# MCG-NJU/LinK

Hardware: AMD Instinct MI355X
Metric: voxels/s through one LinK (3x7)^3 block, 100k active voxels C=64 (higher is better)
Workload: dtype f32

## Files before the change

link_amd/csrc/dense_batch_impl.h:

```cpp
#include <stdlib.h>

#include <type_traits>
#include <vector>

#include "dense_batch_common.h"
#include "dense_gather.h"
#include "dense_io.h"

namespace DC_IO_NS {
using namespace link;

#include "dense_k1_impl.h"
#include "dense_k2_cfg.h"
#include "dense_gather_quad_impl.h"

static_assert(DC_ST_AUX == 16, "the S rows must leave the L2 (sc1) for the in-launch hand-off K1 -> K2");

struct dc_bt_frame_t {
  const void *feats; const int4 *coords; int4 *slots; uint32_t *cnt; int32_t *cell_n; int32_t *vcell; float *S; int32_t *hdr;
  void *out; int64_t n;
};
struct dc_bt_frames_t { dc_bt_frame_t f[DC_BT_MAX]; };
struct dc_bt_par_t {
  const float *w_pre, *pre_ln_w, *pre_ln_b, *w_pos, *ln_w, *ln_b;
// ... 48 lines not shown
    const link_dc_grid_t g = a->g;
    const int n = (int)a->fr.f[f].n;
    const int4 *__restrict__ coords = a->fr.f[f].coords;
    int32_t *__restrict__ vcell = a->fr.f[f].vcell;
    int32_t *__restrict__ hdr = a->fr.f[f].hdr;
    const __amdgpu_buffer_rsrc_t r_slots = dc_rsrc(a->fr.f[f].slots, (uint32_t)((int64_t)g.vp * g.k * 16));
    const __amdgpu_buffer_rsrc_t r_cnt = dc_rsrc(a->fr.f[f].cnt, (uint32_t)(g.vp * 4));
    if (j == 0 && threadIdx.x == 0) hdr[LINK_HDR_NVALID] = n;
    _Pragma("unroll 1") for (int k = 0; k < 4; k++) {
      const int v = (4 * j + k) * 64 + (int)threadIdx.x;
      if (v >= n) break;
      const int4 rc = coords[v];
      const unsigned ux = (unsigned)(floordiv(rc.x, g.s) - g.lo[0]), uy = (unsigned)(floordiv(rc.y, g.s) - g.lo[1]);
      const unsigned uz = (unsigned)(floordiv(rc.z, g.s) - g.lo[2]), ub = (unsigned)(rc.w - g.lo[3]);
      const bool inside = ux < (unsigned)g.dim[0] && uy < (unsigned)g.dim[1] && uz < (unsigned)g.dim[2] && ub < (unsigned)g.dim[3];
      if (!inside) atomicOr(&hdr[LINK_HDR_STATUS_ACC], 1);
      const int pcell = inside ? dc_cell(g, (int)ux, (int)uy, (int)uz, (int)ub) : 0;
      const int rank = __builtin_amdgcn_raw_ptr_buffer_atomic_add_i32(1, r_cnt, pcell ? (uint32_t)pcell * 4u : DC_OOB, 0, 0);
      const bool full = pcell != 0 && rank >= g.k;
      if (full) atomicOr(&hdr[LINK_HDR_STATUS_ACC], 2);
      const bool keep = pcell != 0 && !full;
      st16i_c<true>(r_slots, keep ? dc_slot(g, pcell, rank) * 16u : DC_OOB, make_int4(rc.x, rc.y, rc.z, v));
      vcell[v] = keep ? pcell : 0;
    }
    asm volatile("s_waitcnt vmcnt(0)" ::: "memory");
    if (threadIdx.x == 0) __hip_atomic_fetch_add(&a->sync[bt_ins(f)], 1, __ATOMIC_RELAXED, __HIP_MEMORY_SCOPE_AGENT);
  }
#endif
}

template <int OP, int NB>
__global__ void __launch_bounds__(64 * DC_K1_NW, DC_K1_WAVES) k_dc_batch_k1(dc_bt_frames_t fr, dc_bt_par_t p, link_dc_grid_t g, int nframes,
                                                                           int cpw, int nranges, int wpf, int32_t *__restrict__ sync) {
  constexpr int C = 64;
  extern __shared__ __attribute__((aligned(16))) char smem_raw[];
  const int tid = threadIdx.x, lane = tid & 63;
  bool w_big = false, th_big = false;
  dc_k1_stage<C, OP>(smem_raw, p.w_pre, p.pre_ln_w, p.pre_ln_b, p.w_pos, nullptr, p.cg, 1.0f, g, tid, w_big, th_big);
  w_big = DC_K1_SPLIT ? (__syncthreads_or(w_big) != 0) : (__syncthreads(), false);
  const bool th_slow = DC_THETA_BOUND ? __syncthreads_or(th_big) != 0 : false;
  const int Vi = g.dim[0] * g.dim[1] * g.dim[2] * g.dim[3];
  const int x = (int)(__builtin_amdgcn_s_getreg((4 - 1) << 11 | 0 << 6 | 20) & 7u);
  const int per = (nranges + 7) >> 3;
  const int lo = x * per;
  const int mine = (lo + per < nranges ? lo + per : nranges) - lo;
  if (mine <= 0) return;
  const int total = nframes * mine;
  int32_t *cur = &sync[bt_k1cur(x)];
  int t_next = 0;
  if (lane == 0) t_next = __hip_atomic_fetch_add(cur, 1, __ATOMIC_RELAXED, __HIP_MEMORY_SCOPE_AGENT);
  int pend_f = -1;
  int ins_known = -1;
  for (;;) {
    const int t = __builtin_amdgcn_readfirstlane(t_next);
    if (t >= total) break;
    const unsigned long long tp0 = DC_BT_PROF ? __builtin_amdgcn_s_memrealtime() : 0;
    const int f = t / mine, i = lo + (t - f * mine);
    if (lane == 0) t_next = __hip_atomic_fetch_add(cur, 1, __ATOMIC_RELAXED, __HIP_MEMORY_SCOPE_AGENT);
    const dc_bt_frame_t &F = fr.f[f];
    int ins_a = wpf, ins_b = wpf;
    if (lane == 0) {
      if (f > ins_known) ins_a = __hip_atomic_load(&sync[bt_ins(f)], __ATOMIC_RELAXED, __HIP_MEMORY_SCOPE_AGENT);
      if (f + 1 < nframes && f + 1 > ins_known) ins_b = __hip_atomic_load(&sync[bt_ins(f + 1)], __ATOMIC_RELAXED, __HIP_MEMORY_SCOPE_AGENT);
    }
    const int c_begin = i * cpw;
    const int c_end = (c_begin + cpw < Vi) ? c_begin + cpw : Vi;
    int pc_f, nv_f;
    int4 rf0, rf1, rf2, rf3;
    if (f <= ins_known) dc_k1_prefetch<true>(pc_f, nv_f, rf0, rf1, rf2, rf3, g, F.slots, F.cnt, c_begin, c_end, lane);
    asm volatile("s_waitcnt vmcnt(0)" ::: "memory");
    if (pend_f >= 0 && lane == 0) __hip_atomic_fetch_add(&sync[bt_k1(pend_f)], 1, __ATOMIC_RELAXED, __HIP_MEMORY_SCOPE_AGENT);
    pend_f = f;
    if (f > ins_known) {
      if (__builtin_amdgcn_readfirstlane(ins_a) < wpf && !bt_wait_ge(sync, bt_ins(f), wpf)) return;
      ins_known = f;
      dc_k1_prefetch<true>(pc_f, nv_f, rf0, rf1, rf2, rf3, g, F.slots, F.cnt, c_begin, c_end, lane);
    }
    if (f + 1 < nframes && f + 1 > ins_known && __builtin_amdgcn_readfirstlane(ins_b) >= wpf) ins_known = f + 1;
    if (i == 0 && lane == 0) {
      F.hdr[LINK_HDR_STATUS] = __hip_atomic_load(&F.hdr[LINK_HDR_STATUS_ACC], __ATOMIC_RELAXED, __HIP_MEMORY_SCOPE_AGENT);
      __hip_atomic_store(&F.hdr[LINK_HDR_STATUS_ACC], 0, __ATOMIC_RELAXED, __HIP_MEMORY_SCOPE_AGENT);
    }
    const unsigned long long tp1 = DC_BT_PROF ? __builtin_amdgcn_s_memrealtime() : 0;
    dc_k1_range<C, OP, NB, false, true, DC_BT_K1_WRITEBACK != 0>(smem_raw, F.feats, F.slots, F.cnt, F.cell_n, p.w_pre, 1.0f, p.eps, F.n, g, false, F.S, nullptr,
                                        nullptr, c_begin, c_end, pc_f, nv_f, rf0, rf1, rf2, rf3, w_big, th_slow, i, 0, 0);
    if (DC_BT_PROF && lane == 0) bt_row(p.dbg1, (unsigned long long)f * nranges + i, (unsigned long long)f, (unsigned long long)i, tp0, tp1, __builtin_amdgcn_s_memrealtime(), (unsigned long long)(blockIdx.x * 4 + (tid >> 6)));
  }
  asm volatile("s_waitcnt vmcnt(0)" ::: "memory");
#if DC_BT_RELEASE_FENCE
  __builtin_amdgcn_fence(__ATOMIC_RELEASE, "agent");
  asm volatile("s_waitcnt vmcnt(0)" ::: "memory");
#endif
  if (pend_f >= 0 && lane == 0) __hip_atomic_fetch_add(&sync[bt_k1(pend_f)], 1, __ATOMIC_RELAXED, __HIP_MEMORY_SCOPE_AGENT);
}

struct dc_bt_k2_args_t {
  dc_bt_frames_t fr;
  dc_bt_par_t p;
  link_dc_grid_t g;
  int nframes, txn, tyn, zsplit, nwg, k1_target;
  int32_t *sync;
};

template <int OP, int R>
__global__ void __launch_bounds__(256 + 64 * (DC_K2Q_CW + (DC_K2Q_PMAP ? 1 : 0)), 4) k_dc_batch_k2(dc_bt_k2_args_t args_by_value) {
  (void)args_by_value;
#if defined(__HIP_DEVICE_COMPILE__)
  static_assert(DC_K2Q_PMAP == 1, "the mapper wave draws the items");
  typedef const __attribute__((address_space(4))) dc_bt_k2_args_t *args_ptr_t;
  constexpr unsigned CTL_THREAD = 256 + 64 * DC_K2Q_CW;
  __shared__ int s_ctl[4];
  const int x = (int)(__builtin_amdgcn_s_getreg((4 - 1) << 11 | 0 << 6 | 20) & 7u);
  if (threadIdx.x == CTL_THREAD) {
    args_ptr_t a = (args_ptr_t)__builtin_amdgcn_kernarg_segment_ptr();
    int32_t *sy = a->sync;
    const int per = (a->nwg + 7) >> 3;
    if (DC_BT_PROF)
      bt_row(a->p.dbg2, (unsigned long long)a->nframes * (8 * per) + blockIdx.x, 9999, 0, __builtin_amdgcn_s_memrealtime(), 0, 0, blockIdx.x);
    const int t = __hip_atomic_fetch_add(&sy[bt_cursor(x)], 1, __ATOMIC_RELAXED, __HIP_MEMORY_SCOPE_AGENT);
    s_ctl[2] = __hip_atomic_fetch_add(&sy[bt_cursor(x)], 1, __ATOMIC_RELAXED, __HIP_MEMORY_SCOPE_AGENT);
    s_ctl[3] = x;
    int f = t < a->nframes * per ? t / per : -1;
    if (f >= 0 && !bt_wait_ge(sy, bt_k1(f), a->k1_target)) f = -1;
    s_ctl[0] = f; s_ctl[1] = f >= 0 ? (t - f * per) * 8 + x : 0;
  }
  __syncthreads();
  for (;;) {
    args_ptr_t a = (args_ptr_t)__builtin_amdgcn_kernarg_segment_ptr();
    asm volatile("" : "+s"(a));
    const int f = __builtin_amdgcn_readfirstlane(s_ctl[0]), bid = __builtin_amdgcn_readfirstlane(s_ctl[1]);
    if (f < 0) break;
    const unsigned long long tq0 = DC_BT_PROF ? __builtin_amdgcn_s_memrealtime() : 0;
    __syncthreads();
    {
      const link_dc_grid_t g = a->g;
      unsigned tidx = threadIdx.x;
      asm volatile("" : "+v"(tidx));
      dc_k2q_body<OP, R, false, true>(a->fr.f[f].S, a->fr.f[f].cell_n, a->fr.f[f].slots, a->p.w_pos, nullptr, a->p.ln_w, a->p.ln_b, a->p.cg,
                                      1.0f, a->p.eps, a->fr.f[f].n, g, a->txn, a->tyn, a->zsplit, a->nwg, a->fr.f[f].out, nullptr, bid, tidx);
    }
    if (threadIdx.x == CTL_THREAD) {
      const unsigned long long tq1 = DC_BT_PROF ? __builtin_amdgcn_s_memrealtime() : 0;
      int32_t *sy = a->sync;
      const int per = (a->nwg + 7) >> 3;
      const int t = s_ctl[2], xc = s_ctl[3];
      int fn = t < a->nframes * per ? t / per : -1;
      if (fn >= 0) {
        s_ctl[2] = __hip_atomic_fetch_add(&sy[bt_cursor(xc)], 1, __ATOMIC_RELAXED, __HIP_MEMORY_SCOPE_AGENT);
        if (!bt_wait_ge(sy, bt_k1(fn), a->k1_target)) fn = -1;
      }
      s_ctl[0] = fn; s_ctl[1] = fn >= 0 ? (t - fn * per) * 8 + xc : 0;
      if (DC_BT_PROF) bt_row(a->p.dbg2, (unsigned long long)f * (8 * per) + bid, (unsigned long long)f, (unsigned long long)bid, tq0, tq1, __builtin_amdgcn_s_memrealtime(), (unsigned long long)blockIdx.x);
    }
    __syncthreads();
  }
#endif
}


template <int OP, int R>
static int batch_launch(const dc_bt_host_t &c, const dc_bt_frames_t &fr, const dc_bt_par_t &p, const link_dc_grid_t &g, const link_elk_desc_t &d,
                        int nframes, int64_t nmax, bool strips) {
  using K1 = dc_k1_cfg<64, OP>;
  using KQ = dc_k2q_cfg<OP, R>;
  constexpr int LDS_GRAN = 1280, LDS_GRANS = 128, K1_STATIC = 256, K2_STATIC = 16;
  constexpr int k1_lds = 65 * LDS_GRAN - K1_STATIC;
  constexpr int k2_lds = KQ::LDS_BYTES;
// ... 51 lines not shown
```

link_amd/csrc/dense_fused_impl.h:

```cpp
#pragma once
#include <type_traits>

#include "dense_gather.h"
#include "dense_io.h"

namespace DC_IO_NS {
using namespace link;

#include "dense_k1_impl.h"

template <int C, int OP, int NB, bool PIPE, bool WB = true>
static int launch_k1p(const link_dc_buffers_t *b, const link_dc_grid_t &g, const link_elk_desc_t &d, int64_t n,
                     bool warm, hipStream_t st) {
  using K = dc_k1_cfg<C, OP>;
  const int64_t vi = (int64_t)g.dim[0] * g.dim[1] * g.dim[2] * g.dim[3];
  int64_t waves = (int64_t)(b->tune.k1_wgs > 0 ? b->tune.k1_wgs : 512) * 4;
  int cpw = (int)((vi + waves - 1) / waves);
  if (cpw < 1) cpw = 1;
  const int64_t wgs = (vi + (int64_t)cpw * K::NW - 1) / ((int64_t)cpw * K::NW);
  int k1_pad = b->tune.k1_lds_pad;
  k1_pad = k1_pad < 0 ? 0 : (k1_pad > 16384 ? 16384 : k1_pad);
  const int lds_k1 = K::LDS_BYTES + k1_pad <= 160 * 1024 ? K::LDS_BYTES + k1_pad : K::LDS_BYTES;
  if (lds_k1 > 64 * 1024)
    (void)hipFuncSetAttribute(reinterpret_cast<const void *>(&k_dc_premix_modsum<C, OP, NB, PIPE, WB>),
                              hipFuncAttributeMaxDynamicSharedMemorySize, lds_k1);
  hipLaunchKernelGGL((k_dc_premix_modsum<C, OP, NB, PIPE, WB>), dim3((unsigned)wgs), dim3(64 * K::NW), lds_k1, st, b->feats,
                     reinterpret_cast<int4 *>(b->slots), b->cnt, b->cell_n, b->w_pre, b->pre_ln_w, b->pre_ln_b,
                     b->w_pos, b->alpha, d.cg, d.coord_div, d.eps, n, g, cpw, warm, b->S, b->fin, b->hdr,
                     reinterpret_cast<unsigned long long *>(b->tune.k1_dbg));
  return check_launch("link_dc_premix_modsum");
}

template <int C, int OP, int NB>
static int launch_k1(const link_dc_buffers_t *b, const link_dc_grid_t &g, const link_elk_desc_t &d, int64_t n,
                     bool warm, bool wb, hipStream_t st) {
  if constexpr (C == 64 && NB == 2 && OP != LINK_OP_COSX) {
    if (!wb) return launch_k1p<C, OP, NB, false, false>(b, g, d, n, warm, st);
  }
  return launch_k1p<C, OP, NB, false>(b, g, d, n, warm, st);
}

template <int C, int OP>
static int dispatch_k1_nb(const link_dc_buffers_t *b, const link_dc_grid_t &g, const link_elk_desc_t &d, int64_t n,
                          bool warm, bool wb, hipStream_t st) {
  constexpr int T = C / 16;
  int nb = (d.cg % 16 == 0) ? d.cg / 16 : T;
  if (nb > T) nb = T;
  if (nb == T) return launch_k1<C, OP, T>(b, g, d, n, warm, wb, st);
  if (T >= 2 && nb == T / 2) return launch_k1<C, OP, (T >= 2 ? T / 2 : 1)>(b, g, d, n, warm, wb, st);
  if (T >= 4 && nb == T / 4) return launch_k1<C, OP, (T >= 4 ? T / 4 : 1)>(b, g, d, n, warm, wb, st);
  return launch_k1<C, OP, T>(b, g, d, n, warm, wb, st);
}

template <int C>
static int dispatch_k1_op(const link_dc_buffers_t *b, const link_dc_grid_t &g, const link_elk_desc_t &d, int64_t n,
                          bool warm, bool wb, hipStream_t st) {
  switch (d.op) {
    case LINK_OP_COS: return dispatch_k1_nb<C, LINK_OP_COS>(b, g, d, n, warm, wb, st);
    case LINK_OP_SIN: return dispatch_k1_nb<C, LINK_OP_SIN>(b, g, d, n, warm, wb, st);
    default: return dispatch_k1_nb<C, LINK_OP_COSX>(b, g, d, n, warm, wb, st);
  }
}

#include "dense_fused_mm_impl.h"

template <int LPR, int OP, bool PAIR, bool DIV>
__global__ void __launch_bounds__(256) k_dc_demod(const float *__restrict__ A_, const float *__restrict__ fin,
                                                  const int4 *__restrict__ coords, const int32_t *__restrict__ vcell,
                                                  const float *__restrict__ w_pos, const float *__restrict__ alpha,
                                                  const float *__restrict__ ln_w, const float *__restrict__ ln_b, int c,
                                                  int cg, float coord_div, float eps, int64_t n, int64_t a_rows,
                                                  void *__restrict__ out) {
  constexpr int P = (OP == LINK_OP_COSX) ? 3 : 2;
  constexpr int G = 64 / LPR;
  const int lane = threadIdx.x & 63;
  const int li = lane & (LPR - 1);
  const int ch0 = 4 * li;
  const bool hi = PAIR && (li >= LPR / 2);
  const int ra = P * c * 4;
  const __amdgpu_buffer_rsrc_t r_A = dc_rsrc(A_, (uint32_t)(a_rows * ra));
  const __amdgpu_buffer_rsrc_t r_fin = dc_rsrc(fin, (uint32_t)(n * c * 4));
  const __amdgpu_buffer_rsrc_t r_out = dc_rsrc(out, (uint32_t)(n * c * IO_BYTES));
  float w0[4], w1[4], w2[4], al[4], gw[4], gb[4];
#pragma unroll
  for (int e = 0; e < 4; e++) {
    const int ch = ch0 + e, tc = ch % cg;
    w0[e] = w_pos[3 * tc + 0]; w1[e] = w_pos[3 * tc + 1]; w2[e] = w_pos[3 * tc + 2];
    al[e] = alpha ? alpha[tc] : 1.0f;
    gw[e] = ln_w[ch]; gb[e] = ln_b[ch];
  }
  const float inv_c = 1.0f / (float)c;
  const int64_t npair = (n + 1) >> 1;
  const int64_t ngroups = (int64_t)gridDim.x * 4 * G;
  int64_t p = ((int64_t)blockIdx.x * 4 + (threadIdx.x >> 6)) * G + lane / LPR;
  if (p >= npair) return;
  auto ld_meta = [&](int64_t pp, int4 &ca, int4 &cb, int &va, int &vb) {
    const int64_t q = pp < npair ? pp : npair - 1;
    const int64_t ia = 2 * q, ib = (2 * q + 1 < n) ? 2 * q + 1 : 2 * q;
    ca = coords[ia]; cb = coords[ib];
    va = vcell[ia]; vb = vcell[ib];
  };
  auto ld_rows = [&](int va, int vb, v4i_t (&ra_)[P], v4i_t (&rb_)[P]) {
#pragma unroll
    for (int pp = 0; pp < P; pp++) {
      ra_[pp] = __builtin_amdgcn_raw_buffer_load_b128(r_A, (uint32_t)va * (uint32_t)ra + (uint32_t)((pp * c + ch0) * 4), 0, 0);
      rb_[pp] = __builtin_amdgcn_raw_buffer_load_b128(r_A, (uint32_t)vb * (uint32_t)ra + (uint32_t)((pp * c + ch0) * 4), 0, 0);
    }
  };
  int4 c0a, c0b, c1a, c1b;
  int v0a, v0b, v1a, v1b;
  v4i_t a0[P], b0[P];
  ld_meta(p, c0a, c0b, v0a, v0b);
  ld_rows(v0a, v0b, a0, b0);
  ld_meta(p + ngroups, c1a, c1b, v1a, v1b);
  for (; p < npair; p += ngroups) {
    v4i_t a1[P], b1[P];
    ld_rows(v1a, v1b, a1, b1);
    int4 c2a, c2b;
    int v2a, v2b;
    ld_meta(p + 2 * ngroups, c2a, c2b, v2a, v2b);
    const bool hasB = 2 * p + 1 < n;
    v4i_t fx = {0, 0, 0, 0}, fy = {0, 0, 0, 0};
// ... 846 lines not shown
```

link_amd/csrc/dense_k1_impl.h:

```cpp
#pragma once

#ifndef DC_K1_LCAP
#define DC_K1_LCAP 352
#endif
#ifndef DC_K1_NW
#define DC_K1_NW 4
#endif
#ifndef DC_K1_ABL
#define DC_K1_ABL 0
#endif
#ifndef DC_K1_SPLIT
#define DC_K1_SPLIT 1
#endif
#ifndef DC_K2_ABL
#define DC_K2_ABL 0
#endif
#ifndef DC_K2_SECOND_ROUND
#define DC_K2_SECOND_ROUND 1
#endif
#ifndef DC_K2_PIPE_READS
#define DC_K2_PIPE_READS 0
#endif
#ifndef DC_K1_MFMA32
#define DC_K1_MFMA32 1
// ... 48 lines not shown
#ifndef DC_K1_WAVES
#define DC_K1_WAVES 2
#endif
__device__ __forceinline__ int dc_k1_cell_of(const link_dc_grid_t &g, int chunk, int nrem, int lane) {
  const int q = chunk + (lane < nrem ? lane : 0);
  const int Dx = g.dim[0], Dy = g.dim[1], Dz = g.dim[2];
  const int z = q % Dz;
  int t = q / Dz;
  const int y = t % Dy;
  t /= Dy;
  return dc_cell(g, t % Dx, y, z, t / Dx);
}

template <bool COH = false>
__device__ __forceinline__ void dc_k1_prefetch(int &pc_f, int &nv_f, int4 &rf0, int4 &rf1, int4 &rf2, int4 &rf3,
                                               const link_dc_grid_t &g, const int4 *__restrict__ slots,
                                               const uint32_t *__restrict__ csrc, int c_begin, int c_end, int lane) {
  pc_f = 0; nv_f = 0;
  rf0 = make_int4(0, 0, 0, 0); rf1 = rf0; rf2 = rf0; rf3 = rf0;
  if (c_begin < c_end) {
    pc_f = dc_k1_cell_of(g, c_begin, (c_end - c_begin < 64) ? c_end - c_begin : 64, lane);
    const __amdgpu_buffer_rsrc_t r_slots = dc_rsrc(slots, (uint32_t)((int64_t)g.vp * g.k * 16));
    const __amdgpu_buffer_rsrc_t r_c = dc_rsrc(csrc, (uint32_t)(g.vp * 4));
    rf0 = ld16i_c<COH>(r_slots, slots, (uint32_t)pc_f * DC_INL + 0); rf1 = ld16i_c<COH>(r_slots, slots, (uint32_t)pc_f * DC_INL + 1);
    rf2 = ld16i_c<COH>(r_slots, slots, (uint32_t)pc_f * DC_INL + 2); rf3 = ld16i_c<COH>(r_slots, slots, (uint32_t)pc_f * DC_INL + 3);
    nv_f = ld4i_c<COH>(r_c, csrc, (uint32_t)pc_f);
  }
}

template <int C, int OP>
__device__ __forceinline__ void dc_k1_stage(char *smem_raw, const float *__restrict__ w_pre, const float *__restrict__ ln_w,
                                            const float *__restrict__ ln_b, const float *__restrict__ w_pos,
                                            const float *__restrict__ alpha, int cg, float coord_div, const link_dc_grid_t &g,
                                            int tid, bool &w_big, bool &th_big) {
  using K = dc_k1_cfg<C, OP>;
  constexpr int LDW = K::LDW;
  float *w_lds = reinterpret_cast<float *>(smem_raw);
  float *ln_lds = reinterpret_cast<float *>(smem_raw + K::WIMG_BYTES);
  float *pw_lds = ln_lds + 2 * C;
  (void)w_lds;
  {
    constexpr int NF4 = C * C / 4;
    constexpr int NT = 64 * K::NW;
    constexpr int NV = (NF4 + NT - 1) / NT;
    float4 wv[NV];
#pragma unroll
    for (int i = 0; i < NV; i++) {
      const int e = (i * NT + tid) * 4;
      wv[i] = *reinterpret_cast<const float4 *>(&w_pre[(NF4 % NT == 0 || e < C * C) ? e : 0]);
    }
#pragma unroll
    for (int i = 0; i < NV; i++) {
      int e = (i * NT + tid) * 4;
      if (NF4 % NT != 0 && e >= C * C) e = 0;
      const int r = e / C, col = e - r * C;
      const float4 wq = (NF4 % NT == 0 || (i * NT + tid) * 4 < C * C) ? wv[i] : *reinterpret_cast<const float4 *>(&w_pre[0]);
      if constexpr (DC_K1_SPLIT) {
        uint2 hi, lo;
        dc_split4(wq, hi, lo);
        unsigned short *wh = reinterpret_cast<unsigned short *>(smem_raw);
        *reinterpret_cast<uint2 *>(&wh[r * K::LDH + col]) = hi;
        *reinterpret_cast<uint2 *>(&wh[r * K::LDH + C + col]) = lo;
        w_big |= !(fmaxf(fmaxf(fabsf(wq.x), fabsf(wq.y)), fmaxf(fabsf(wq.z), fabsf(wq.w))) < 32768.0f);
      } else {
        *reinterpret_cast<float4 *>(&w_lds[r * LDW + col]) = wq;
      }
    }
    if (tid < C) ln_lds[tid] = ln_w[tid];
    else if (tid < 2 * C) ln_lds[tid] = ln_b[tid - C];
    if (tid < C) {
      const int tc = tid % cg;
      const float q0 = w_pos[3 * tc + 0], q1 = w_pos[3 * tc + 1], q2 = w_pos[3 * tc + 2], qa = alpha ? alpha[tc] : 1.0f;
      pw_lds[tid] = q0; pw_lds[C + tid] = q1; pw_lds[2 * C + tid] = q2;
      pw_lds[3 * C + tid] = qa;
      if (DC_THETA_BOUND) {
        float ax, ay, az;
        dc_coord_absmax(g, coord_div, ax, ay, az);
        th_big = dc_theta_leaves_fast_range(ax, ay, az, q0, q1, q2, qa);
      }
    }
  }
}

template <int C, int OP, int NB, bool PIPE, bool COH = false, bool WB = true>
__device__ __forceinline__ void dc_k1_range(char *smem_raw, const void *__restrict__ feats, int4 *__restrict__ slots,
                                            uint32_t *__restrict__ cnt, int32_t *__restrict__ cell_n,
                                            const float *__restrict__ w_pre, float coord_div, float eps, int64_t n,
                                            const link_dc_grid_t &g, bool warm, float *__restrict__ S_, float *__restrict__ fin,
                                            unsigned long long *__restrict__ dbg, int c_begin,
                                            int c_end, const int pc_f, const int nv_f, const int4 rf0, const int4 rf1, const int4 rf2,
                                            const int4 rf3, bool w_big, bool th_slow, int wid,
                                            unsigned long long tq0, unsigned long long tq1) {
  using K = dc_k1_cfg<C, OP>;
  constexpr int T = K::T, P = K::P, LDW = K::LDW;
  unsigned long long tq_cell = 0, tq_fill = 0, tq_body = 0, tq_sum = 0;
  int tq_tiles = 0;
  float *w_lds = reinterpret_cast<float *>(smem_raw);
  float *ln_lds = reinterpret_cast<float *>(smem_raw + K::WIMG_BYTES);
  float *pw_lds = ln_lds + 2 * C;
  const int tid = threadIdx.x, lane = tid & 63, wave = __builtin_amdgcn_readfirstlane(tid >> 6);
  const int li = lane & 15, gq = lane >> 4;
  char *wbase = smem_raw + K::W_BYTES + wave * K::WAVE_BYTES;
  int4 *list = reinterpret_cast<int4 *>(wbase + K::LIST_OFF);
  int *scell = reinterpret_cast<int *>(wbase + K::SCELL_OFF);
  char *xbuf = wbase + K::X_OFF;
  const uint32_t *__restrict__ csrc = warm ? reinterpret_cast<const uint32_t *>(cell_n) : cnt;
  const __amdgpu_buffer_rsrc_t r_S = dc_rsrc(S_, (uint32_t)((g.vp + 1) * K::RB));
  const __amdgpu_buffer_rsrc_t r_fin = dc_rsrc(fin, (uint32_t)(n * C * 4));
  const __amdgpu_buffer_rsrc_t r_slots = dc_rsrc(slots, (uint32_t)((int64_t)g.vp * g.k * 16));
  const __amdgpu_buffer_rsrc_t r_n = dc_rsrc(cell_n, (uint32_t)(g.vp * 4));
  const __amdgpu_buffer_rsrc_t r_cnt = dc_rsrc(cnt, (uint32_t)(g.vp * 4));
  const int rl = lane;
  const bool ract = rl < K::RGL;

  for (int chunk = c_begin; chunk < c_end;) {
    const int nrem = (c_end - chunk < 64) ? c_end - chunk : 64;
    unsigned long long tqa = dbg ? DC_NOW() : 0;
    int pc, nv;
    int4 r0, r1, r2, r3;
    if (chunk == c_begin) {
      pc = pc_f; nv = nv_f; r0 = rf0; r1 = rf1; r2 = rf2; r3 = rf3;
    } else {
      pc = dc_k1_cell_of(g, chunk, nrem, lane);
      r0 = ld16i_c<COH>(r_slots, slots, (uint32_t)pc * DC_INL + 0); r1 = ld16i_c<COH>(r_slots, slots, (uint32_t)pc * DC_INL + 1);
      r2 = ld16i_c<COH>(r_slots, slots, (uint32_t)pc * DC_INL + 2); r3 = ld16i_c<COH>(r_slots, slots, (uint32_t)pc * DC_INL + 3);
      nv = ld4i_c<COH>(warm ? r_n : r_cnt, csrc, (uint32_t)pc);
    }
    constexpr int LCAPX = K::LCAP;
    nv = nv < g.k ? nv : g.k;
    nv = nv < LCAPX ? nv : LCAPX;
    if (lane >= nrem) nv = 0;
    int incl = nv;
    incl += __builtin_amdgcn_update_dpp(0, incl, 0x111, 0xF, 0xF, true);
    incl += __builtin_amdgcn_update_dpp(0, incl, 0x112, 0xF, 0xF, true);
    incl += __builtin_amdgcn_update_dpp(0, incl, 0x114, 0xF, 0xF, true);
    incl += __builtin_amdgcn_update_dpp(0, incl, 0x118, 0xF, 0xF, true);
    {
      const int t0 = __builtin_amdgcn_readlane(incl, 15), t1 = __builtin_amdgcn_readlane(incl, 31), t2 = __builtin_amdgcn_readlane(incl, 47);
      incl += gq == 0 ? 0 : (gq == 1 ? t0 : (gq == 2 ? t0 + t1 : t0 + t1 + t2));
    }
    const unsigned long long fit = __ballot(lane < nrem && incl <= LCAPX);
    const int nfit = __builtin_amdgcn_readfirstlane(__popcll(fit));
    const int Ttot = __builtin_amdgcn_readlane(incl, nfit - 1);
    int4 rs[4] = {r0, r1, r2, r3};
    if (lane < nfit) {
      const int excl = incl - nv;
      int k0 = nv > 0 ? r0.w * 4 + 0 : INT_MAX, k1 = nv > 1 ? r1.w * 4 + 1 : INT_MAX;
      int k2 = nv > 2 ? r2.w * 4 + 2 : INT_MAX, k3 = nv > 3 ? r3.w * 4 + 3 : INT_MAX;
      int a, bb;
      a = min(k0, k1); bb = max(k0, k1); k0 = a; k1 = bb;
      a = min(k2, k3); bb = max(k2, k3); k2 = a; k3 = bb;
      a = min(k0, k2); bb = max(k0, k2); k0 = a; k2 = bb;
      a = min(k1, k3); bb = max(k1, k3); k1 = a; k3 = bb;
      a = min(k1, k2); bb = max(k1, k2); k1 = a; k2 = bb;
      const int ks[4] = {k0, k1, k2, k3};
#pragma unroll
      for (int j = 0; j < 4; j++) {
        const int s = ks[j] & 3;
        int4 r;
        r.x = s == 0 ? r0.x : (s == 1 ? r1.x : (s == 2 ? r2.x : r3.x));
        r.y = s == 0 ? r0.y : (s == 1 ? r1.y : (s == 2 ? r2.y : r3.y));
        r.z = s == 0 ? r0.z : (s == 1 ? r1.z : (s == 2 ? r2.z : r3.z));
        r.w = ks[j] >> 2;
        if (j < nv) { list[excl + j] = r; scell[excl + j] = pc; }
        rs[j] = r;
      }
      for (int k = DC_INL; k < nv; k++) {
        const int4 r = ld16i_c<COH>(r_slots, slots, dc_slot(g, pc, k));
        scell[excl + k] = pc;
        int pos = k;
        while (pos > 0 && list[excl + pos - 1].w > r.w) {
          list[excl + pos] = list[excl + pos - 1];
          pos--;
        }
        list[excl + pos] = r;
      }
      if constexpr (WB) {
        if (nv > DC_INL && !warm)
          for (int k = 0; k < nv; k++) st16i_c<COH>(r_slots, dc_slot(g, pc, k) * 16u, list[excl + k]);
      }
    }
    auto publish = [&]() {
      if constexpr (WB) {
#pragma unroll
        for (int j = 0; j < 4; j++)
          st16i_c<COH>(r_slots, (lane < nfit && j < nv && nv <= DC_INL && !warm) ? ((uint32_t)pc * DC_INL + j) * 16u : DC_OOB, rs[j]);
      }
      const uint32_t coff = (lane < nfit && !warm) ? (uint32_t)pc * 4u : DC_OOB;
      st4i_c<COH>(r_n, coff, nv);
      st4i(r_cnt, coff, 0);
    };
    auto publish_empty = [&]() {
      for (unsigned long long em = __ballot(lane < nfit && nv == 0); em; em &= em - 1) {
        const int pcj = __builtin_amdgcn_readlane(pc, __builtin_ctzll(em));
        st16(r_S, ract ? (uint32_t)pcj * (uint32_t)K::RB + (uint32_t)rl * 16u : DC_OOB, make_float4(0.f, 0.f, 0.f, 0.f));
      }
    };
    if constexpr (!DC_K1_LATE_PUBLISH) { publish(); publish_empty(); }
    __builtin_amdgcn_wave_barrier();
    asm volatile("s_waitcnt lgkmcnt(0)" ::: "memory");
    if (dbg) { const unsigned long long tqb = DC_NOW(); tq_cell += tqb - tqa; tqa = tqb; }
    const int ntile = (Ttot + 15) >> 4;
    const int nloop = ntile;
    float4 acc = make_float4(0.f, 0.f, 0.f, 0.f);
    auto ld_rows = [&](int tile_idx, int4 &rr, float4 (&ff)[T]) {
      int sl = 16 * tile_idx + li;
      sl = sl < Ttot ? sl : Ttot - 1;
      rr = list[sl];
#pragma unroll
      for (int tt = 0; tt < T; tt++)
        ff[tt] = io_ld4(feats, (int64_t)((DC_K1_ABL & 8) ? li : rr.w) * C + 16 * tt + 4 * gq);
    };
    auto mfma_tile = [&](const float4 (&ff)[T], floatx4 (&cc)[T]) {
      if (DC_K1_ABL & 1) {
#pragma unroll
        for (int tp = 0; tp < T; tp++) cc[tp] = (floatx4){ff[tp].x, ff[tp].y, ff[tp].z, ff[tp].w};
        return;
      }
#pragma unroll
      for (int tp = 0; tp < T; tp++) cc[tp] = (floatx4){0.f, 0.f, 0.f, 0.f};
      if constexpr (DC_K1_SPLIT) {
        uint2 bh[T], bl[T];
        float mx = 0.f;
#pragma unroll
        for (int tt = 0; tt < T; tt++) {
          dc_split4(ff[tt], bh[tt], bl[tt]);
          mx = fmaxf(mx, fmaxf(fmaxf(fabsf(ff[tt].x), fabsf(ff[tt].y)), fmaxf(fabsf(ff[tt].z), fabsf(ff[tt].w))));
        }
        if (__builtin_expect(!(w_big || __any(!(mx < 32768.0f))), 1)) {
          const unsigned short *wh = reinterpret_cast<const unsigned short *>(smem_raw);
          if constexpr (DC_K1_MFMA32 && T % 2 == 0) {
#pragma unroll
            for (int tt = 0; tt < T; tt += 2) {
              uint2 ah[2][T], al[2][T];
#pragma unroll
              for (int h = 0; h < 2; h++)
#pragma unroll
                for (int tp = 0; tp < T; tp++) {
                  ah[h][tp] = *reinterpret_cast<const uint2 *>(&wh[(16 * tp + li) * K::LDH + 16 * (tt + h) + 4 * gq]);
                  al[h][tp] = *reinterpret_cast<const uint2 *>(&wh[(16 * tp + li) * K::LDH + C + 16 * (tt + h) + 4 * gq]);
                }
#pragma unroll
              for (int tp = 0; tp < T; tp++) cc[tp] = dc_mfma_f16x2(al[0][tp], al[1][tp], bh[tt], bh[tt + 1], cc[tp]);
              if constexpr (IO != 1) {
#pragma unroll
                for (int tp = 0; tp < T; tp++) cc[tp] = dc_mfma_f16x2(ah[0][tp], ah[1][tp], bl[tt], bl[tt + 1], cc[tp]);
              }
#pragma unroll
              for (int tp = 0; tp < T; tp++) cc[tp] = dc_mfma_f16x2(ah[0][tp], ah[1][tp], bh[tt], bh[tt + 1], cc[tp]);
            }
            return;
          }
#pragma unroll
          for (int tt = 0; tt < T; tt++) {
            uint2 ah[T], al[T];
#pragma unroll
            for (int tp = 0; tp < T; tp++) {
              ah[tp] = *reinterpret_cast<const uint2 *>(&wh[(16 * tp + li) * K::LDH + 16 * tt + 4 * gq]);
              al[tp] = *reinterpret_cast<const uint2 *>(&wh[(16 * tp + li) * K::LDH + C + 16 * tt + 4 * gq]);
            }
#pragma unroll
            for (int tp = 0; tp < T; tp++) cc[tp] = dc_mfma_f16(al[tp], bh[tt], cc[tp]);
            if constexpr (IO != 1) {
#pragma unroll
              for (int tp = 0; tp < T; tp++) cc[tp] = dc_mfma_f16(ah[tp], bl[tt], cc[tp]);
            }
#pragma unroll
            for (int tp = 0; tp < T; tp++) cc[tp] = dc_mfma_f16(ah[tp], bh[tt], cc[tp]);
          }
          return;
        }
      }
#pragma unroll
      for (int tt = 0; tt < T; tt++) {
        float4 a[T];
#pragma unroll
        for (int tp = 0; tp < T; tp++) {
          if constexpr (DC_K1_SPLIT) a[tp] = *reinterpret_cast<const float4 *>(&w_pre[(16 * tp + li) * C + 16 * tt + 4 * gq]);
          else a[tp] = *reinterpret_cast<const float4 *>(&w_lds[(16 * tp + li) * LDW + 16 * tt + 4 * gq]);
        }
#pragma unroll
        for (int tp = 0; tp < T; tp++) cc[tp] = __builtin_amdgcn_mfma_f32_16x16x4f32(a[tp].x, ff[tt].x, cc[tp], 0, 0, 0);
#pragma unroll
        for (int tp = 0; tp < T; tp++) cc[tp] = __builtin_amdgcn_mfma_f32_16x16x4f32(a[tp].y, ff[tt].y, cc[tp], 0, 0, 0);
#pragma unroll
        for (int tp = 0; tp < T; tp++) cc[tp] = __builtin_amdgcn_mfma_f32_16x16x4f32(a[tp].z, ff[tt].z, cc[tp], 0, 0, 0);
#pragma unroll
        for (int tp = 0; tp < T; tp++) cc[tp] = __builtin_amdgcn_mfma_f32_16x16x4f32(a[tp].w, ff[tt].w, cc[tp], 0, 0, 0);
      }
    };
    int4 recA = make_int4(0, 0, 0, 0), recB = recA, recC = recA;
    float4 fA[T], fB[T];
    floatx4 acA[T], acB[T];
    if (ntile > 0) {
      ld_rows(0, recA, PIPE ? fB : fA);
      ld_rows(ntile > 1 ? 1 : 0, recB, PIPE ? fA : fB);
      if constexpr (DC_K1_LATE_PUBLISH) publish();
      mfma_tile(PIPE ? fB : fA, acA);
    } else {
      if constexpr (DC_K1_LATE_PUBLISH) publish();
    }
    if constexpr (DC_K1_LATE_PUBLISH) publish_empty();
    if (dbg) { const unsigned long long tqb = DC_NOW(); tq_fill += tqb - tqa; tqa = tqb; }
    auto step = [&](auto phase_tag, int t, const int4 &rec, const int4 &recn, int4 &rec2, const float4 (&fn)[T], float4 (&f2)[T],
                    const floatx4 (&ac)[T], floatx4 (&acn)[T]) {
      constexpr int PHASE = decltype(phase_tag)::value;
      if (PHASE != 2 && ntile > 0) {
        const int slot = 16 * t + li;
        float x = (float)rec.x, y = (float)rec.y, z = (float)rec.z;
        if (coord_div != 1.0f) { x = x / coord_div; y = y / coord_div; z = z / coord_div; }
        float th[NB][4];
        bool big = false;
#pragma unroll
        for (int tb = 0; tb < NB; tb++) {
          const float4 q0 = *reinterpret_cast<const float4 *>(&pw_lds[16 * tb + 4 * gq]);
          const float4 q1 = *reinterpret_cast<const float4 *>(&pw_lds[C + 16 * tb + 4 * gq]);
          const float4 q2 = *reinterpret_cast<const float4 *>(&pw_lds[2 * C + 16 * tb + 4 * gq]);
          const float4 qa = *reinterpret_cast<const float4 *>(&pw_lds[3 * C + 16 * tb + 4 * gq]);
          th[tb][0] = theta_of(x, y, z, q0.x, q1.x, q2.x, qa.x); th[tb][1] = theta_of(x, y, z, q0.y, q1.y, q2.y, qa.y);
          th[tb][2] = theta_of(x, y, z, q0.z, q1.z, q2.z, qa.z); th[tb][3] = theta_of(x, y, z, q0.w, q1.w, q2.w, qa.w);
          if (!DC_THETA_BOUND) {
#pragma unroll
            for (int r = 0; r < 4; r++) big |= !(fabsf(th[tb][r]) < 32768.0f);
          }
        }
        const bool slow = DC_THETA_BOUND ? th_slow : __any(big);
        const bool more = PIPE && t + 1 < ntile;
        (void)recn;
        auto body = [&](auto more_tag, auto slow_tag) {
          constexpr bool MORE = decltype(more_tag)::value, SLOW = decltype(slow_tag)::value;
          if constexpr (MORE) mfma_tile(fn, acn);
          if constexpr (MORE) ld_rows(t + 2 < ntile ? t + 2 : t + 1, rec2, f2);
          float sn[NB][4], cs[NB][4];
#pragma unroll
          for (int tb = 0; tb < NB; tb++)
#pragma unroll
            for (int r = 0; r < 4; r++) {
              if (DC_K1_ABL & 2) { sn[tb][r] = th[tb][r]; cs[tb][r] = 1.0f - th[tb][r]; }
              else if constexpr (SLOW) sincos_nocall(th[tb][r], sn[tb][r], cs[tb][r]);
              else sincos_small(th[tb][r], sn[tb][r], cs[tb][r]);
            }
          float s = 0.f;
#pragma unroll
          for (int tp = 0; tp < T; tp++) s += (ac[tp][0] + ac[tp][1]) + (ac[tp][2] + ac[tp][3]);
          s = dc_k1_sum_groups(s);
          const float mean = s * (1.0f / C);
          float qq = 0.f;
#pragma unroll
          for (int tp = 0; tp < T; tp++)
#pragma unroll
            for (int r = 0; r < 4; r++) {
              const float d = ac[tp][r] - mean;
              qq += d * d;
            }
          qq = dc_k1_sum_groups(qq);
          const float rstd = 1.0f / sqrtf(qq * (1.0f / C) + eps);
#pragma unroll
          for (int tp = 0; tp < T; tp++) {
            const float4 lw = *reinterpret_cast<const float4 *>(&ln_lds[16 * tp + 4 * gq]);
            const float4 lb = *reinterpret_cast<const float4 *>(&ln_lds[C + 16 * tp + 4 * gq]);
            const float fv[4] = {(ac[tp][0] - mean) * rstd * lw.x + lb.x, (ac[tp][1] - mean) * rstd * lw.y + lb.y,
                                 (ac[tp][2] - mean) * rstd * lw.z + lb.z, (ac[tp][3] - mean) * rstd * lw.w + lb.w};
            if (OP == LINK_OP_COSX)
              st16(r_fin, slot < Ttot ? (uint32_t)rec.w * (uint32_t)(C * 4) + (uint32_t)((16 * tp + 4 * gq) * 4) : DC_OOB,
                   make_float4(fv[0], fv[1], fv[2], fv[3]));
            const int tb = tp % NB;
            float p0[4], p1[4], p2[4];
#pragma unroll
            for (int r = 0; r < 4; r++) {
              if (OP == LINK_OP_SIN) { p0[r] = fv[r] * sn[tb][r]; p1[r] = fv[r] * cs[tb][r]; }
              else { p0[r] = fv[r] * cs[tb][r]; p1[r] = fv[r] * sn[tb][r]; }
              p2[r] = fv[r] * th[tb][r];
            }
            char *xr = xbuf + li * K::XROW + (16 * tp + 4 * gq) * 4;
            *reinterpret_cast<float4 *>(xr) = make_float4(p0[0], p0[1], p0[2], p0[3]);
            *reinterpret_cast<float4 *>(xr + C * 4) = make_float4(p1[0], p1[1], p1[2], p1[3]);
            if (P == 3) *reinterpret_cast<float4 *>(xr + 2 * C * 4) = make_float4(p2[0], p2[1], p2[2], p2[3]);
          }
          if constexpr (MORE && !SLOW) {
#pragma unroll
            for (int i = 0; i < T * T * 4; i++) {
              __builtin_amdgcn_sched_group_barrier(0x008, 1, 0);
              __builtin_amdgcn_sched_group_barrier(0x002, 6, 0);
            }
          }
        };
        if (__builtin_expect(slow, 0)) {
          if (more) {
            mfma_tile(fn, acn);
            ld_rows(t + 2 < ntile ? t + 2 : t + 1, rec2, f2);
          }
          body(std::false_type{}, std::true_type{});
        } else {
          if (more) body(std::true_type{}, std::false_type{}); else body(std::false_type{}, std::false_type{});
        }
        __builtin_amdgcn_wave_barrier();
        asm volatile("s_waitcnt lgkmcnt(0)" ::: "memory");
      }
      if (PHASE != 2 && dbg) { const unsigned long long tqb = DC_NOW(); tq_body += tqb - tqa; tqa = tqb; tq_tiles++; }
      if (PHASE == 1 || (DC_K1_ABL & 4)) return;
      {
        const int slot = 16 * t + li;
        const int myc = slot < Ttot ? scell[slot] : -1;
        const int nxc = slot + 1 < Ttot ? scell[slot + 1] : -2;
        const unsigned closes = (unsigned)__ballot(gq == 0 && slot < Ttot && myc != nxc);
        const char *xrow = xbuf + (ract ? rl : 0) * 16;
#pragma unroll
        for (int h = 0; h < 16; h += DC_K1_SUMB) {
          float4 v[DC_K1_SUMB];
#pragma unroll
          for (int k = 0; k < DC_K1_SUMB; k++) v[k] = *reinterpret_cast<const float4 *>(xrow + (h + k) * K::XROW);
#pragma unroll
          for (int k = 0; k < DC_K1_SUMB; k++) {
            if (16 * t + h + k < Ttot) {
              acc.x += v[k].x; acc.y += v[k].y; acc.z += v[k].z; acc.w += v[k].w;
              if ((closes >> (h + k)) & 1u) {
                const int pcs = __builtin_amdgcn_readlane(myc, h + k);
                st16(r_S, ract ? (uint32_t)pcs * (uint32_t)K::RB + (uint32_t)rl * 16u : DC_OOB, acc);
                acc = make_float4(0.f, 0.f, 0.f, 0.f);
              }
            }
          }
        }
      }
      __builtin_amdgcn_wave_barrier();
      if (dbg) { const unsigned long long tqb = DC_NOW(); tq_sum += tqb - tqa; tqa = tqb; }
    };
    if constexpr (PIPE) {
      for (int t = 0; t < nloop; t += 2) {
        step(std::integral_constant<int, 0>{}, t, recA, recB, recC, fA, fB, acA, acB);
        recA = recB; recB = recC;
        if (t + 1 < nloop) {
          step(std::integral_constant<int, 0>{}, t + 1, recA, recB, recC, fB, fA, acB, acA);
          recA = recB; recB = recC;
        }
      }
    } else {
      using body_only = std::integral_constant<int, 1>;
      using sums_only = std::integral_constant<int, 2>;
      for (int t = 0; t < nloop; t += 2) {
        if (t > 0) {
          if (t + 1 < ntile) ld_rows(t + 1, recB, fB);
          mfma_tile(fA, acA);
        }
        if (t > 0) step(sums_only{}, t - 1, recB, recB, recC, fB, fB, acA, acB);
        step(body_only{}, t, recA, recB, recC, fB, fB, acA, acB);
        if (t + 1 < nloop) {
          if (t + 2 < ntile) ld_rows(t + 2, recA, fA);
          mfma_tile(fB, acA);
          step(sums_only{}, t, recA, recA, recC, fA, fA, acA, acB);
          step(body_only{}, t + 1, recB, recA, recC, fA, fA, acA, acB);
        }
      }
      if (nloop > 0) step(sums_only{}, nloop - 1, recA, recA, recC, fA, fA, acA, acB);
    }
    chunk += nfit;
  }
  if (dbg && lane == 0) {
    unsigned long long *d = dbg + (size_t)wid * 8;
    const unsigned long long te = DC_NOW();
    d[0] = tq1 - tq0; d[1] = tq_cell; d[2] = tq_fill; d[3] = tq_body; d[4] = tq_sum; d[5] = te - tq0; d[6] = tq_tiles; d[7] = tq0;
  }
}

template <int C, int OP, int NB, bool PIPE, bool WB = true>
__global__ void __launch_bounds__(64 * DC_K1_NW, PIPE ? 2 : DC_K1_WAVES) k_dc_premix_modsum(
    const void *__restrict__ feats, int4 *__restrict__ slots, uint32_t *__restrict__ cnt,
    int32_t *__restrict__ cell_n, const float *__restrict__ w_pre, const float *__restrict__ ln_w,
    const float *__restrict__ ln_b, const float *__restrict__ w_pos, const float *__restrict__ alpha, int cg,
    float coord_div, float eps, int64_t n, link_dc_grid_t g, int cpw, bool warm, float *__restrict__ S_,
    float *__restrict__ fin, int32_t *__restrict__ hdr, unsigned long long *__restrict__ dbg) {
  using K = dc_k1_cfg<C, OP>;
  DC_PROF_PTR(dbg);
  unsigned long long tq0 = dbg ? DC_NOW() : 0, tq1 = 0;
  extern __shared__ __attribute__((aligned(16))) char smem_raw[];
  const int tid = threadIdx.x, lane = tid & 63, wave = __builtin_amdgcn_readfirstlane(tid >> 6);
  const int Vi = g.dim[0] * g.dim[1] * g.dim[2] * g.dim[3];
  const int wid = blockIdx.x * K::NW + wave;
  const int c_begin = wid * cpw;
  const int c_end = (c_begin + cpw < Vi) ? c_begin + cpw : Vi;
  int pc_f, nv_f;
  int4 rf0, rf1, rf2, rf3;
  dc_k1_prefetch<false>(pc_f, nv_f, rf0, rf1, rf2, rf3, g, slots, warm ? reinterpret_cast<const uint32_t *>(cell_n) : cnt, c_begin, c_end, lane);
  bool w_big = false;
  bool th_big = false;
  dc_k1_stage<C, OP>(smem_raw, w_pre, ln_w, ln_b, w_pos, alpha, cg, coord_div, g, tid, w_big, th_big);
  if (blockIdx.x == 0 && tid == 0 && !warm) {
    hdr[LINK_HDR_STATUS] = hdr[LINK_HDR_STATUS_ACC];
    hdr[LINK_HDR_STATUS_ACC] = 0;
  }
  w_big = DC_K1_SPLIT ? (__syncthreads_or(w_big) != 0 || (LINK_COSX_EXACT && OP == LINK_OP_COSX)) : (__syncthreads(), false);
  const bool th_slow = DC_THETA_BOUND ? __syncthreads_or(th_big) != 0 : false;
  if (dbg) tq1 = DC_NOW();
  if (c_begin >= c_end) return;
  dc_k1_range<C, OP, NB, PIPE, false, WB>(smem_raw, feats, slots, cnt, cell_n, w_pre, coord_div, eps, n, g, warm, S_, fin, dbg, c_begin,
                                       c_end, pc_f, nv_f, rf0, rf1, rf2, rf3, w_big, th_slow, wid, tq0, tq1);
}
```

Before: 3.275 billion.

## Replace K1 tile loop with three-deep row prefetch and drop PIPE variant

Removes the PIPE template parameter and its alternate loop. The non-pipelined schedule becomes a single loop that keeps three row records in flight (recA/recB/recC) and alternates two feature buffers. Each iteration finishes the current tile, issues the next MFMA, runs the sums for the finished tile, and prefetches the rows two tiles ahead, so load latency overlaps with compute. It also drops the second accumulator array and the sched_group_barrier interleaving hints. ld_rows is now called with tile indices past ntile (t+3, t+4, and 1 or 2 when ntile is 1), so correctness relies on ld_rows guarding out-of-range slots. The extra loads may cost a little bandwidth.

```diff
diff --git a/link_amd/csrc/dense_batch_impl.h b/link_amd/csrc/dense_batch_impl.h
--- a/link_amd/csrc/dense_batch_impl.h
+++ b/link_amd/csrc/dense_batch_impl.h
@@ -154,7 +154,7 @@
       __hip_atomic_store(&F.hdr[LINK_HDR_STATUS_ACC], 0, __ATOMIC_RELAXED, __HIP_MEMORY_SCOPE_AGENT);
     }
     const unsigned long long tp1 = DC_BT_PROF ? __builtin_amdgcn_s_memrealtime() : 0;
-    dc_k1_range<C, OP, NB, false, true, DC_BT_K1_WRITEBACK != 0>(smem_raw, F.feats, F.slots, F.cnt, F.cell_n, p.w_pre, 1.0f, p.eps, F.n, g, false, F.S, nullptr,
+    dc_k1_range<C, OP, NB, true, DC_BT_K1_WRITEBACK != 0>(smem_raw, F.feats, F.slots, F.cnt, F.cell_n, p.w_pre, 1.0f, p.eps, F.n, g, false, F.S, nullptr,
                                         nullptr, c_begin, c_end, pc_f, nv_f, rf0, rf1, rf2, rf3, w_big, th_slow, i, 0, 0);
     if (DC_BT_PROF && lane == 0) bt_row(p.dbg1, (unsigned long long)f * nranges + i, (unsigned long long)f, (unsigned long long)i, tp0, tp1, __builtin_amdgcn_s_memrealtime(), (unsigned long long)(blockIdx.x * 4 + (tid >> 6)));
   }
diff --git a/link_amd/csrc/dense_fused_impl.h b/link_amd/csrc/dense_fused_impl.h
--- a/link_amd/csrc/dense_fused_impl.h
+++ b/link_amd/csrc/dense_fused_impl.h
@@ -9,7 +9,7 @@
 
 #include "dense_k1_impl.h"
 
-template <int C, int OP, int NB, bool PIPE, bool WB = true>
+template <int C, int OP, int NB, bool WB = true>
 static int launch_k1p(const link_dc_buffers_t *b, const link_dc_grid_t &g, const link_elk_desc_t &d, int64_t n,
                      bool warm, hipStream_t st) {
   using K = dc_k1_cfg<C, OP>;
@@ -22,9 +22,9 @@
   k1_pad = k1_pad < 0 ? 0 : (k1_pad > 16384 ? 16384 : k1_pad);
   const int lds_k1 = K::LDS_BYTES + k1_pad <= 160 * 1024 ? K::LDS_BYTES + k1_pad : K::LDS_BYTES;
   if (lds_k1 > 64 * 1024)
-    (void)hipFuncSetAttribute(reinterpret_cast<const void *>(&k_dc_premix_modsum<C, OP, NB, PIPE, WB>),
+    (void)hipFuncSetAttribute(reinterpret_cast<const void *>(&k_dc_premix_modsum<C, OP, NB, WB>),
                               hipFuncAttributeMaxDynamicSharedMemorySize, lds_k1);
-  hipLaunchKernelGGL((k_dc_premix_modsum<C, OP, NB, PIPE, WB>), dim3((unsigned)wgs), dim3(64 * K::NW), lds_k1, st, b->feats,
+  hipLaunchKernelGGL((k_dc_premix_modsum<C, OP, NB, WB>), dim3((unsigned)wgs), dim3(64 * K::NW), lds_k1, st, b->feats,
                      reinterpret_cast<int4 *>(b->slots), b->cnt, b->cell_n, b->w_pre, b->pre_ln_w, b->pre_ln_b,
                      b->w_pos, b->alpha, d.cg, d.coord_div, d.eps, n, g, cpw, warm, b->S, b->fin, b->hdr,
                      reinterpret_cast<unsigned long long *>(b->tune.k1_dbg));
@@ -35,9 +35,9 @@
 static int launch_k1(const link_dc_buffers_t *b, const link_dc_grid_t &g, const link_elk_desc_t &d, int64_t n,
                      bool warm, bool wb, hipStream_t st) {
   if constexpr (C == 64 && NB == 2 && OP != LINK_OP_COSX) {
-    if (!wb) return launch_k1p<C, OP, NB, false, false>(b, g, d, n, warm, st);
-  }
-  return launch_k1p<C, OP, NB, false>(b, g, d, n, warm, st);
+    if (!wb) return launch_k1p<C, OP, NB, false>(b, g, d, n, warm, st);
+  }
+  return launch_k1p<C, OP, NB>(b, g, d, n, warm, st);
 }
 
 template <int C, int OP>
diff --git a/link_amd/csrc/dense_k1_impl.h b/link_amd/csrc/dense_k1_impl.h
--- a/link_amd/csrc/dense_k1_impl.h
+++ b/link_amd/csrc/dense_k1_impl.h
@@ -154,7 +154,7 @@
   }
 }
 
-template <int C, int OP, int NB, bool PIPE, bool COH = false, bool WB = true>
+template <int C, int OP, int NB, bool COH = false, bool WB = true>
 __device__ __forceinline__ void dc_k1_range(char *smem_raw, const void *__restrict__ feats, int4 *__restrict__ slots,
                                             uint32_t *__restrict__ cnt, int32_t *__restrict__ cell_n,
                                             const float *__restrict__ w_pre, float coord_div, float eps, int64_t n,
@@ -273,7 +273,6 @@
     asm volatile("s_waitcnt lgkmcnt(0)" ::: "memory");
     if (dbg) { const unsigned long long tqb = DC_NOW(); tq_cell += tqb - tqa; tqa = tqb; }
     const int ntile = (Ttot + 15) >> 4;
-    const int nloop = ntile;
     float4 acc = make_float4(0.f, 0.f, 0.f, 0.f);
     auto ld_rows = [&](int tile_idx, int4 &rr, float4 (&ff)[T]) {
       int sl = 16 * tile_idx + li;
@@ -363,21 +362,20 @@
     };
     int4 recA = make_int4(0, 0, 0, 0), recB = recA, recC = recA;
     float4 fA[T], fB[T];
-    floatx4 acA[T], acB[T];
+    floatx4 acA[T];
     if (ntile > 0) {
-      ld_rows(0, recA, PIPE ? fB : fA);
-      ld_rows(ntile > 1 ? 1 : 0, recB, PIPE ? fA : fB);
+      ld_rows(0, recA, fA);
+      ld_rows(1, recB, fB);
       if constexpr (DC_K1_LATE_PUBLISH) publish();
-      mfma_tile(PIPE ? fB : fA, acA);
+      mfma_tile(fA, acA);
     } else {
       if constexpr (DC_K1_LATE_PUBLISH) publish();
     }
     if constexpr (DC_K1_LATE_PUBLISH) publish_empty();
+    if (ntile > 0) ld_rows(2, recC, fA);
     if (dbg) { const unsigned long long tqb = DC_NOW(); tq_fill += tqb - tqa; tqa = tqb; }
-    auto step = [&](auto phase_tag, int t, const int4 &rec, const int4 &recn, int4 &rec2, const float4 (&fn)[T], float4 (&f2)[T],
-                    const floatx4 (&ac)[T], floatx4 (&acn)[T]) {
-      constexpr int PHASE = decltype(phase_tag)::value;
-      if (PHASE != 2 && ntile > 0) {
+    auto finish = [&](int t, const int4 &rec, const floatx4 (&ac)[T]) {
+      {
         const int slot = 16 * t + li;
         float x = (float)rec.x, y = (float)rec.y, z = (float)rec.z;
         if (coord_div != 1.0f) { x = x / coord_div; y = y / coord_div; z = z / coord_div; }
@@ -397,12 +395,8 @@
           }
         }
         const bool slow = DC_THETA_BOUND ? th_slow : __any(big);
-        const bool more = PIPE && t + 1 < ntile;
-        (void)recn;
-        auto body = [&](auto more_tag, auto slow_tag) {
-          constexpr bool MORE = decltype(more_tag)::value, SLOW = decltype(slow_tag)::value;
-          if constexpr (MORE) mfma_tile(fn, acn);
-          if constexpr (MORE) ld_rows(t + 2 < ntile ? t + 2 : t + 1, rec2, f2);
+        auto body = [&](auto slow_tag) {
+          constexpr bool SLOW = decltype(slow_tag)::value;
           float sn[NB][4], cs[NB][4];
 #pragma unroll
           for (int tb = 0; tb < NB; tb++)
@@ -449,28 +443,16 @@
             *reinterpret_cast<float4 *>(xr + C * 4) = make_float4(p1[0], p1[1], p1[2], p1[3]);
             if (P == 3) *reinterpret_cast<float4 *>(xr + 2 * C * 4) = make_float4(p2[0], p2[1], p2[2], p2[3]);
           }
-          if constexpr (MORE && !SLOW) {
-#pragma unroll
-            for (int i = 0; i < T * T * 4; i++) {
-              __builtin_amdgcn_sched_group_barrier(0x008, 1, 0);
-              __builtin_amdgcn_sched_group_barrier(0x002, 6, 0);
-            }
-          }
         };
-        if (__builtin_expect(slow, 0)) {
-          if (more) {
-            mfma_tile(fn, acn);
-            ld_rows(t + 2 < ntile ? t + 2 : t + 1, rec2, f2);
-          }
-          body(std::false_type{}, std::true_type{});
-        } else {
-          if (more) body(std::true_type{}, std::false_type{}); else body(std::false_type{}, std::false_type{});
-        }
+        if (__builtin_expect(slow, 0)) body(std::true_type{});
+        else body(std::false_type{});
         __builtin_amdgcn_wave_barrier();
         asm volatile("s_waitcnt lgkmcnt(0)" ::: "memory");
       }
-      if (PHASE != 2 && dbg) { const unsigned long long tqb = DC_NOW(); tq_body += tqb - tqa; tqa = tqb; tq_tiles++; }
-      if (PHASE == 1 || (DC_K1_ABL & 4)) return;
+      if (dbg) { const unsigned long long tqb = DC_NOW(); tq_body += tqb - tqa; tqa = tqb; tq_tiles++; }
+    };
+    auto sums = [&](int t) {
+      if (DC_K1_ABL & 4) return;
       {
         const int slot = 16 * t + li;
         const int myc = slot < Ttot ? scell[slot] : -1;
@@ -498,33 +480,24 @@
       __builtin_amdgcn_wave_barrier();
       if (dbg) { const unsigned long long tqb = DC_NOW(); tq_sum += tqb - tqa; tqa = tqb; }
     };
-    if constexpr (PIPE) {
-      for (int t = 0; t < nloop; t += 2) {
-        step(std::integral_constant<int, 0>{}, t, recA, recB, recC, fA, fB, acA, acB);
-        recA = recB; recB = recC;
-        if (t + 1 < nloop) {
-          step(std::integral_constant<int, 0>{}, t + 1, recA, recB, recC, fB, fA, acB, acA);
-          recA = recB; recB = recC;
-        }
-      }
-    } else {
-      using body_only = std::integral_constant<int, 1>;
-      using sums_only = std::integral_constant<int, 2>;
-      for (int t = 0; t < nloop; t += 2) {
-        if (t > 0) {
-          if (t + 1 < ntile) ld_rows(t + 1, recB, fB);
-          mfma_tile(fA, acA);
-        }
-        if (t > 0) step(sums_only{}, t - 1, recB, recB, recC, fB, fB, acA, acB);
-        step(body_only{}, t, recA, recB, recC, fB, fB, acA, acB);
-        if (t + 1 < nloop) {
-          if (t + 2 < ntile) ld_rows(t + 2, recA, fA);
-          mfma_tile(fB, acA);
-          step(sums_only{}, t, recA, recA, recC, fA, fA, acA, acB);
-          step(body_only{}, t + 1, recB, recA, recC, fA, fA, acA, acB);
-        }
-      }
-      if (nloop > 0) step(sums_only{}, nloop - 1, recA, recA, recC, fA, fA, acA, acB);
+    if (ntile > 0) {
+      int t = 0;
+      for (; t + 1 < ntile; t += 2) {
+        finish(t, recA, acA);
+        recA = recC;
+        mfma_tile(fB, acA);
+        sums(t);
+        ld_rows(t + 3, recC, fB);
+        finish(t + 1, recB, acA);
+        recB = recC;
+        if (t + 2 < ntile) mfma_tile(fA, acA);
+        sums(t + 1);
+        ld_rows(t + 4, recC, fA);
+      }
+      if (t < ntile) {
+        finish(t, recA, acA);
+        sums(t);
+      }
     }
     chunk += nfit;
   }
@@ -535,8 +508,8 @@
   }
 }
 
-template <int C, int OP, int NB, bool PIPE, bool WB = true>
-__global__ void __launch_bounds__(64 * DC_K1_NW, PIPE ? 2 : DC_K1_WAVES) k_dc_premix_modsum(
+template <int C, int OP, int NB, bool WB = true>
+__global__ void __launch_bounds__(64 * DC_K1_NW, DC_K1_WAVES) k_dc_premix_modsum(
     const void *__restrict__ feats, int4 *__restrict__ slots, uint32_t *__restrict__ cnt,
     int32_t *__restrict__ cell_n, const float *__restrict__ w_pre, const float *__restrict__ ln_w,
     const float *__restrict__ ln_b, const float *__restrict__ w_pos, const float *__restrict__ alpha, int cg,
@@ -565,6 +538,6 @@
   const bool th_slow = DC_THETA_BOUND ? __syncthreads_or(th_big) != 0 : false;
   if (dbg) tq1 = DC_NOW();
   if (c_begin >= c_end) return;
-  dc_k1_range<C, OP, NB, PIPE, false, WB>(smem_raw, feats, slots, cnt, cell_n, w_pre, coord_div, eps, n, g, warm, S_, fin, dbg, c_begin,
+  dc_k1_range<C, OP, NB, false, WB>(smem_raw, feats, slots, cnt, cell_n, w_pre, coord_div, eps, n, g, warm, S_, fin, dbg, c_begin,
                                        c_end, pc_f, nv_f, rf0, rf1, rf2, rf3, w_big, th_slow, wid, tq0, tq1);
 }
```

After: 3.323 billion (median of 6 runs). No clear change (+1.4%).
